# fonzcastellanos/scalable-video-codec

Measured on AMD Instinct MI355X. Metric: encoded frames/sec (1080p, 16x16 HBMA+DCT), higher is better.
Workload: dtype u8 (SAD, integer argmin) / f64 accumulate -> f32 (DCT, quant)

## Files before the change

include/svc/clip_encoder.hpp:

```cpp
#ifndef SVC_CLIP_ENCODER_HPP
#define SVC_CLIP_ENCODER_HPP

#include <cstdint>
#include <functional>
#include <memory>

#include "svc_hip.h"

namespace svc {

struct Shard {
  uint32_t first_frame = 0;
  uint32_t frames = 0;
  bool needs_halo = false;
  uint32_t pairs = 0;
  uint32_t first_encoded = 0;
};

Shard PlanShard(uint32_t clip_frames, uint32_t world, uint32_t rank);

enum class Schedule : uint32_t { kSerial = 0, kPipelined = 1 };

struct ClipEncoderConfig {
  uint32_t width = 0, height = 0;
  uint32_t levels = 3;
  uint32_t mv_block = 16;
  uint32_t search_range = 8;
  uint32_t dct_block_w = 8, dct_block_h = 8;
  uint32_t fg_step = 1, bg_step = 640;
  bool wire = false;
  bool compact = false;
  bool segmentation = true;
  uint64_t seed = 0;
  svc_ransac_params ransac{1, 7.5f, 0.99f, 0.5f};
  svc_segment_params segment{3, 3, 10, 3, 10, 1.0f, 4};
  uint32_t clip_frames = 0;
  uint32_t rank = 0, world = 1;
  Schedule schedule = Schedule::kPipelined;
  uint32_t hbma_flags = SVC_HBMA_AUTO;
  uint32_t lat_depth = 0;
  bool standalone_shapes = false;
  bool segment_fork = false;
  bool inline_rmse = false;
  bool narrow_attempts = false;
  bool two_bgr_passes = false;
  bool always_speculate = false;
  bool keep_foreground_prior = false;
  uint32_t chunk_pairs = 0;
  bool whole_shard_steps = false;
  bool idle_rule_any_size = false;
  bool fork_behind_front = false;
  bool random_policy = false;
  bool mixed_steps = false;
  bool search_after_transform = false;
};

enum class Stage : uint32_t { kLumaPyramid = 0, kHalo, kHbma, kRansac, kSegment, kTransform, kTypePatch, kCount };
enum class Buffer : uint32_t { kMv = 0, kMinMad, kGlobalMotion, kRmse, kInlierMask, kInlierCount, kBlockTypes,
                               kCoeffs, kRecords, kPyramids, kBgr,
                               kCompact , kCompactOffsets ,
                               kCompactChoice , kCount };

class ClipEncoder {
 public:
  using HaloFn = std::function<void(const uint8_t* d_send, uint8_t* d_recv, uint64_t bytes, void* stream)>;

  explicit ClipEncoder(const ClipEncoderConfig& config);
  ~ClipEncoder();
  ClipEncoder(const ClipEncoder&) = delete;
  ClipEncoder& operator=(const ClipEncoder&) = delete;

  const Shard& shard() const;
  uint32_t padded_width() const;
  uint32_t padded_height() const;
  uint32_t blocks() const;
  uint64_t pyramid_stride() const;

  void LoadFrames(const uint8_t* src, uint32_t first_local, uint32_t n, bool src_on_device);

  void SetComm(void* nccl_comm);
  void SetHaloTransport(HaloFn fn);

  void Step(bool timed = false);
  uint32_t StepFrames(const uint8_t* device_frames, bool timed = false);
  void WaitStep(uint32_t step);
  void SetCompactBudget(const svc_step_pair* ladder, uint32_t ladder_len, uint32_t bytes_per_frame);
  void Flush();
  void Sync();

  void StageTime(Stage s, double* total_ms, uint32_t* launches);
  uint64_t StagePairs(Stage s);
  void ResetTimers();
  uint32_t steps_submitted() const;
  uint32_t chunks_per_step() const;
  uint32_t output_sets() const;

  void ResetPolicy();
  void PolicyInfo(uint64_t* chunks_decided, uint64_t* chunks_speculated, double* foreground_share);

  void* Output(Buffer b, uint64_t* bytes);

 private:
  struct Impl;
  std::unique_ptr<Impl> p_;
  void StepOn(const uint8_t* frames, bool timed);
};

// ... 4 lines not shown
```

include/svc_clip.h:

```cpp
#ifndef SVC_CLIP_H
#define SVC_CLIP_H

#include <stdint.h>

#include "svc_hip.h"

#ifdef __cplusplus
extern "C" {
#endif

typedef struct svc_clip svc_clip;

#define SVC_CLIP_SERIAL 0u
#define SVC_CLIP_PIPELINED 1u

#define SVC_CLIP_TUNE_STANDALONE_SHAPES 1u
#define SVC_CLIP_TUNE_SEGMENT_FORK 2u
#define SVC_CLIP_TUNE_INLINE_RMSE 8u
#define SVC_CLIP_TUNE_NARROW_ATTEMPTS 4u
#define SVC_CLIP_TUNE_TWO_BGR_PASSES 16u
#define SVC_CLIP_TUNE_ALWAYS_SPECULATE 32u
#define SVC_CLIP_KEEP_FOREGROUND_PRIOR 64u
#define SVC_CLIP_OUTPUT_COMPACT 8192u
#define SVC_CLIP_TUNE_IDLE_RULE_ANY_SIZE 512u
#define SVC_CLIP_TUNE_FORK_BEHIND_FRONT 4096u
#define SVC_CLIP_TUNE_RANDOM_POLICY 2048u
#define SVC_CLIP_TUNE_MIXED_STEPS 1024u
#define SVC_CLIP_TUNE_SEARCH_AFTER_TRANSFORM 256u
#define SVC_CLIP_TUNE_WHOLE_SHARD_STEPS 128u

typedef struct svc_clip_config {
  uint32_t struct_size;
  uint32_t width, height;
  uint32_t levels, mv_block, search_range;
  uint32_t dct_block_w, dct_block_h;
  uint32_t fg_step, bg_step;
  uint32_t wire;
  uint32_t segmentation;
  uint64_t seed;
  svc_ransac_params ransac;
  svc_segment_params segment;
  uint32_t clip_frames;
  uint32_t rank, world;
  uint32_t schedule;
  uint32_t chunk_pairs;
  uint32_t hbma_flags;
  uint32_t lat_depth;
  uint32_t tuning;
} svc_clip_config;

typedef struct svc_clip_info {
  uint32_t padded_w, padded_h, mv_field_w, mv_field_h, blocks, ransac_iters;
  uint64_t pyramid_stride, frame_bytes, record_bytes;
  uint32_t first_frame, frames, pairs, first_encoded, needs_halo;
  uint32_t chunks_per_step;
  uint32_t output_sets;
  uint32_t reserved;
} svc_clip_info;

enum { SVC_STAGE_LUMA_PYRAMID = 0, SVC_STAGE_HALO, SVC_STAGE_HBMA, SVC_STAGE_RANSAC, SVC_STAGE_SEGMENT,
       SVC_STAGE_TRANSFORM, SVC_STAGE_TYPE_PATCH ,
       SVC_STAGE_COUNT };
enum { SVC_BUF_MV = 0, SVC_BUF_MIN_MAD, SVC_BUF_GLOBAL_MOTION, SVC_BUF_RMSE, SVC_BUF_INLIER_MASK,
       SVC_BUF_INLIER_COUNT, SVC_BUF_BLOCK_TYPES, SVC_BUF_COEFFS, SVC_BUF_RECORDS, SVC_BUF_PYRAMIDS,
       SVC_BUF_BGR, SVC_BUF_COMPACT , SVC_BUF_COMPACT_OFFSETS,
       SVC_BUF_COMPACT_CHOICE , SVC_BUF_COUNT };

typedef int (*svc_clip_halo_fn)(const uint8_t* d_send, uint8_t* d_recv, uint64_t bytes, void* stream,
                                void* user);

const char* svc_clip_last_error(void);

int svc_clip_plan_shard(uint32_t clip_frames, uint32_t world, uint32_t rank, uint32_t* first_frame,
                        uint32_t* frames, uint32_t* pairs, uint32_t* first_encoded);

int svc_clip_create(const svc_clip_config* config, svc_clip** out);
void svc_clip_destroy(svc_clip* clip);
int svc_clip_get_info(svc_clip* clip, svc_clip_info* out);

int svc_clip_load_frames(svc_clip* clip, const uint8_t* src, uint32_t first_local, uint32_t n,
                         int src_on_device);

// ... 27 lines not shown
```

scalable_video_codec_amd/clip.py:

```python
from __future__ import annotations

import ctypes as C
import os
from typing import Callable, Dict, Optional, Tuple

import torch

from . import native
from .configs import CodecConfig
from .native import RansacParams, SegmentParams

_vp, _u32, _u64 = C.c_void_p, C.c_uint32, C.c_uint64

SERIAL, PIPELINED = 0, 1
TUNE_STANDALONE_SHAPES, TUNE_SEGMENT_FORK, TUNE_NARROW_ATTEMPTS, TUNE_INLINE_RMSE, TUNE_TWO_BGR_PASSES, TUNE_ALWAYS_SPECULATE = 1, 2, 4, 8, 16, 32
TUNE_IDLE_RULE_ANY_SIZE = 512
TUNE_FORK_BEHIND_FRONT = 4096
TUNE_RANDOM_POLICY = 2048
TUNE_MIXED_STEPS = 1024
TUNE_SEARCH_AFTER_TRANSFORM = 256
TUNE_WHOLE_SHARD_STEPS = 128
OUTPUT_COMPACT = 8192
KEEP_FOREGROUND_PRIOR = 64
STAGES = ("luma_pyramid", "halo_exchange", "hbma", "ransac", "segment", "dct_quant", "type_patch")
BUFFERS = {"mv": (0, torch.float32), "min_mad": (1, torch.float32), "global_motion": (2, torch.float32),
           "rmse": (3, torch.float32), "inlier_mask": (4, torch.uint8), "inlier_count": (5, torch.int32),
           "block_types": (6, torch.int32), "coeffs": (7, torch.float32), "records": (8, torch.uint8),
           "pyramids": (9, torch.uint8), "bgr": (10, torch.uint8), "compact": (11, torch.uint8), "compact_offsets": (12, torch.int64),
           "compact_choice": (13, torch.int32)}
COMM_ID_BYTES = 128


class ClipConfig(C.Structure):
    _fields_ = [("struct_size", _u32), ("width", _u32), ("height", _u32), ("levels", _u32), ("mv_block", _u32), ("search_range", _u32),
                ("dct_block_w", _u32), ("dct_block_h", _u32), ("fg_step", _u32), ("bg_step", _u32), ("wire", _u32),
                ("segmentation", _u32), ("seed", _u64), ("ransac", RansacParams), ("segment", SegmentParams),
                ("clip_frames", _u32), ("rank", _u32), ("world", _u32), ("schedule", _u32), ("chunk_pairs", _u32),
                ("hbma_flags", _u32), ("lat_depth", _u32), ("tuning", _u32)]


class ClipInfo(C.Structure):
    _fields_ = [(n, _u32) for n in ("padded_w", "padded_h", "mv_field_w", "mv_field_h", "blocks", "ransac_iters")] + \
               [(n, _u64) for n in ("pyramid_stride", "frame_bytes", "record_bytes")] + \
               [(n, _u32) for n in ("first_frame", "frames", "pairs", "first_encoded", "needs_halo", "chunks_per_step", "output_sets", "reserved")]


HALO_FN = C.CFUNCTYPE(C.c_int, _vp, _vp, _u64, _vp, _vp)

SIGNATURES = {
    "svc_clip_last_error": (C.c_char_p, []),
    "svc_clip_plan_shard": (C.c_int, [_u32, _u32, _u32] + [C.POINTER(_u32)] * 4),
    "svc_clip_create": (C.c_int, [C.POINTER(ClipConfig), C.POINTER(_vp)]),
    "svc_clip_destroy": (None, [_vp]),
    "svc_clip_get_info": (C.c_int, [_vp, C.POINTER(ClipInfo)]),
    "svc_clip_load_frames": (C.c_int, [_vp, _vp, _u32, _u32, C.c_int]),
    "svc_clip_set_comm": (C.c_int, [_vp, _vp]),
    "svc_clip_set_halo_callback": (C.c_int, [_vp, HALO_FN, _vp]),
    "svc_clip_step": (C.c_int, [_vp, C.c_int]),
    "svc_clip_step_frames": (C.c_int, [_vp, _vp, C.c_int, C.POINTER(_u32)]),
    "svc_clip_wait_step": (C.c_int, [_vp, _u32]),
    "svc_clip_set_compact_budget": (C.c_int, [_vp, C.POINTER(native.StepPair), _u32, _u32]),
    "svc_clip_flush": (C.c_int, [_vp]),
    "svc_clip_sync": (C.c_int, [_vp]),
    "svc_clip_stage_time": (C.c_int, [_vp, _u32, C.POINTER(C.c_double), C.POINTER(_u32)]),
    "svc_clip_stage_pairs": (C.c_int, [_vp, _u32, C.POINTER(_u64)]),
    "svc_clip_reset_timers": (C.c_int, [_vp]),
    "svc_clip_reset_policy": (C.c_int, [_vp]),
    "svc_clip_policy_info": (C.c_int, [_vp, C.POINTER(_u64), C.POINTER(_u64), C.POINTER(C.c_double)]),
    "svc_clip_output": (C.c_int, [_vp, _u32, C.POINTER(_vp), C.POINTER(_u64)]),
    "svc_clip_read": (C.c_int, [_vp, _u32, _u64, _vp, _u64, C.c_int]),
}

_lib: Optional[C.CDLL] = None

# ... 211 lines not shown
```

scalable_video_codec_amd/csrc/host/clip_encoder.cpp:

```cpp
#include "svc/clip_encoder.hpp"

#include <algorithm>
#include <cstring>
#include <stdexcept>
#include <string>
#include <utility>
#include <vector>

#include "encode_geometry.hpp"
#include "hip_raii.hpp"
#include "svc_clip.h"

namespace svc {
namespace {

using namespace host;

constexpr Who kWho{"svc::ClipEncoder"};
void Hip(hipError_t e, const char* what) { kWho.Hip(e, what); }
void Abi(int rc, const char* what) { kWho.Abi(rc, what); }
bool Ready(hipEvent_t e) { return kWho.Ready(e); }

constexpr uint32_t kStages = (uint32_t)Stage::kCount;

}

Shard PlanShard(uint32_t clip_frames, uint32_t world, uint32_t rank) {
  Shard s;
  if (world == 0 || rank >= world) return s;
  const uint32_t base = clip_frames / world, extra = clip_frames % world;
  s.frames = base + (rank < extra ? 1u : 0u);
  s.first_frame = rank * base + std::min(rank, extra);
  s.needs_halo = s.first_frame > 0 && s.frames > 0;
  s.pairs = s.frames == 0 ? 0 : s.frames - (s.needs_halo ? 0u : 1u);
  s.first_encoded = s.needs_halo ? s.first_frame : s.first_frame + 1;
  return s;
}

struct ClipEncoder::Impl : EncodeGeometry {
  ClipEncoderConfig c;
  Shard sh;
  uint32_t iters = 0;
  uint64_t record_bytes = 0, seg_ws_bytes = 0;
  static constexpr int kMaxDepth = 3, kSets = kMaxDepth + 2;
  int depth = 1, nsets = 1;
  uint32_t nch = 1, cp = 0;
  struct Micro { uint32_t step = 0, p0 = 0, pn = 0; bool first = true; uint8_t order = 0; const uint8_t* frames = nullptr; };
  static constexpr int kRing = 8;
  Micro ring[kRing], next_micro;
  uint32_t n_steps = 0;
  const uint8_t* step_frames = nullptr;
  Event e_step[kRing];
  uint64_t step_last_micro[kRing] = {};
  void MarkStepDone(uint64_t d) {
    const uint32_t s = StepOf(d);
    if (step_last_micro[s % kRing] == d) Hip(hipEventRecord(e_step[s % kRing], sM), "hipEventRecord");
  }
  const Micro& At(uint64_t m) const { return ring[(int)(m % (uint64_t)kRing)]; }
  uint32_t StepOf(uint64_t m) const { return At(m).step; }
  uint32_t P0(uint64_t m) const { return At(m).p0; }
  uint32_t Pn(uint64_t m) const { return At(m).pn; }
  int Slot(uint64_t m) const { return (int)(m % (uint64_t)nsets); }
  DevBuf<uint8_t> bgr, pyr[2], mask[kSets], seg_ws[kMaxDepth], records[kSets + 1];
  DevBuf<float> mv[kSets], mad[kSets], gm[kSets], rmse[kSets], coeffs[kSets + 1];
  DevBuf<uint8_t> redo_ws[kMaxDepth];
  DevBuf<uint32_t> count[kSets], types[kSets], samples;
  DevBuf<uint8_t> compact, compact_ws;
  DevBuf<uint64_t> compact_off;
  std::vector<svc_step_pair> budget_ladder;
  DevBuf<uint32_t> compact_budget, compact_choice;
  Event e_pyr[2], e_halo[2], e_fork, e_join[kSets], e_rfork, e_rmse[kSets];
  bool halo_recorded[2] = {false, false}, join_pending[kSets] = {}, rmse_pending[kSets] = {};
  bool defer_rmse = false;
  uint64_t iter = 0, fork_iter[kSets] = {};
  void* comm = nullptr;
  HaloFn halo;
  uint64_t n_luma = 0, n_hbma = 0, n_lat = 0, n_dct = 0;
  uint32_t lat_flags = 0;
  bool fused_records = false;
  bool one_bgr_pass = false;
  int rec_sets = 1;
  DevBuf<uint8_t>& Records(uint64_t m) { return records[(int)(StepOf(m) % (uint32_t)rec_sets)]; }
  bool spec_quant = false;
  int coeff_sets = 1;
  DevBuf<float>& Coeffs(uint64_t m) { return coeffs[coeff_sets > 1 ? (int)(StepOf(m) % (uint32_t)coeff_sets) : 0]; }
  bool GrowCoeffSets() {
    if (coeff_sets == rec_sets) return true;
    while (n_dct < n_luma) Iterate(false, last_timed);
    for (int b = 1; b < rec_sets; ++b)
      if (!coeffs[b].TryAlloc(coeffs[0].n)) {
        for (int k = 1; k < b; ++k) coeffs[k].Free();
        spec_quant = false;
        return false;
      }
    coeff_sets = rec_sets;
    return true;
  }
  bool spec_step[kSets + 1] = {};
  bool& SpecStep(uint64_t m) { return spec_step[(int)(m % (uint64_t)(kSets + 1))]; }
  static constexpr int kFgSlots = 8;
  static constexpr double kSpecMaxShare = 0.02;
  static constexpr uint64_t kSpecMinPixels = 50000000ull;
  static constexpr uint64_t kChunkMinPixels = 300000000ull;
  static constexpr uint64_t kIdleRuleMinPixels = 400000000ull;
  static constexpr uint32_t kMaxAutoChunks = 1;
  DevBuf<uint32_t> fg_dev;
  PinBuf<uint32_t> fg_host;
  Event e_fg[kFgSlots];
  bool fg_pending[kFgSlots] = {};
  uint64_t fg_blocks[kFgSlots] = {};
  uint64_t n_fg = 0;
  double fg_share = -1.0;
  uint64_t n_spec = 0, n_decided = 0;
  void MeasureForeground(uint64_t m, hipStream_t st) {
    if (!spec_quant || c.two_bgr_passes || c.always_speculate || !Pn(m)) return;
    const int slot = (int)(n_fg % kFgSlots);
    if (fg_pending[slot] && !Ready(e_fg[slot])) return;
    Abi(svc_hip_count_foreground(types[Set(m)].p + (uint64_t)P0(m) * blocks, (uint64_t)Pn(m) * blocks, fg_dev.p + slot, st), "svc_hip_count_foreground");
    Hip(hipMemcpyAsync(fg_host.p + slot, fg_dev.p + slot, 4, hipMemcpyDeviceToHost, st), "hipMemcpyAsync");
    Hip(hipEventRecord(e_fg[slot], st), "hipEventRecord");
    fg_pending[slot] = true;
    fg_blocks[slot] = (uint64_t)Pn(m) * blocks;
    ++n_fg;
  }
  void PollForeground() {
// ... 22 lines not shown
  bool WouldReadOnce() {
    if (one_bgr_pass) return true;
    if (!spec_quant || c.two_bgr_passes) return false;
    if (c.always_speculate) return true;
    PollForeground();
    return fg_share >= 0.0 && fg_share <= kSpecMaxShare;
  }
  void ResetPolicy() {
    fg_share = -1.0;
    n_fg = 0;
    for (bool& p : fg_pending) p = false;
  }
  bool last_timed = false;
  std::vector<std::pair<Event, Event>> timed[kStages];
  std::vector<Event> event_pool;

  Event TimingEvent() {
    if (event_pool.empty()) return Event(kWho, true);
    Event e = std::move(event_pool.back());
    event_pool.pop_back();
    return e;
  }

  uint64_t timed_pairs[kStages] = {};
  uint64_t cur_pairs = 0;
  template <typename F> void Run(Stage st, hipStream_t stream, bool timing, F&& fn) {
    if (!timing) { fn(); return; }
    timed_pairs[(uint32_t)st] += cur_pairs;
    Event a = TimingEvent(), b = TimingEvent();
    Hip(hipEventRecord(a, stream), "hipEventRecord");
    fn();
    Hip(hipEventRecord(b, stream), "hipEventRecord");
    timed[(uint32_t)st].emplace_back(std::move(a), std::move(b));
  }

  int Par(uint64_t m) const { return c.schedule == Schedule::kPipelined ? (int)(StepOf(m) & 1u) : 0; }
  int Set(uint64_t m) const { return (int)(StepOf(m) % (uint32_t)nsets); }

  uint32_t Skip() const { return sh.needs_halo ? 0u : 1u; }
  bool decided = false;
  void Decide(uint64_t m) {
    if (At(m).order && spec_quant && Pn(m)) {
      decided = At(m).order == 2;
      ++n_decided;
      n_spec += decided;
      return;
    }
    decided = spec_quant && Pn(m) && DecideSpeculation(m);
    if (decided && coeff_sets != rec_sets && (!At(m).first || !GrowCoeffSets())) {
      decided = false;
      --n_spec;
    }
  }
  template <typename Between> void Luma(uint64_t m, hipStream_t st, bool timing, Between&& between) {
    cur_pairs = Pn(m);
    const int b = Par(m);
    const uint32_t p0 = P0(m), pn = Pn(m), skip = Skip();
    const bool first_chunk = At(m).first;
    if (spec_quant) SpecStep(m) = pn ? decided : false;
    if (pn && (one_bgr_pass || (spec_quant && SpecStep(m)))) {
      const uint8_t* enc = At(m).frames + (uint64_t)(skip + p0) * frame_bytes;
      uint8_t* slots = pyr[b].p + (uint64_t)(1 + skip + p0) * pyr_stride;
      Run(Stage::kTransform, st, timing, [&] {
        if (!one_bgr_pass)
          Abi(svc_hip_dct_quant_luma_frames(enc, frame_bytes, pn, pw, ph, c.dct_block_w, c.bg_step,
                                            Coeffs(m).p + (uint64_t)p0 * 3 * plane_elems, slots, pyr_stride, st), "svc_hip_dct_quant_luma_frames");
        else
          Abi(svc_hip_dct_records_luma_frames(enc, frame_bytes, pn, pw, ph, c.dct_block_w, ph,
                                              Records(m).p + (uint64_t)p0 * record_bytes, record_bytes, slots, pyr_stride, st), "svc_hip_dct_records_luma_frames");
      });
      between();
      cur_pairs = pn;
      Run(Stage::kLumaPyramid, st, timing, [&] {
        if (skip && first_chunk)
          Abi(svc_hip_luma_pyramid_frames(At(m).frames, frame_bytes, 1, pw, ph, c.levels, pyr[b].p + pyr_stride, pyr_stride, st),
              "svc_hip_luma_pyramid_frames");
        Abi(svc_hip_pyramid_levels_frames(slots, pyr_stride, pn, pw, ph, c.levels, st), "svc_hip_pyramid_levels_frames");
      });
      return;
    }
    const uint32_t f0 = first_chunk ? 0u : p0 + skip, f1 = p0 + pn + skip;
    if (f1 <= f0) return;
    Run(Stage::kLumaPyramid, st, timing, [&] {
      Abi(svc_hip_luma_pyramid_frames(At(m).frames + (uint64_t)f0 * frame_bytes, frame_bytes, f1 - f0, pw, ph, c.levels,
                                      pyr[b].p + (uint64_t)(1 + f0) * pyr_stride, pyr_stride, st), "svc_hip_luma_pyramid_frames");
    });
  }

  void Halo(uint64_t m, bool timing) {
    cur_pairs = 0;
    const int b = Par(m);
    Hip(hipEventRecord(e_pyr[b], sM), "hipEventRecord");
    Hip(hipStreamWaitEvent(sC, e_pyr[b], 0), "hipStreamWaitEvent");
    Run(Stage::kHalo, sC, timing, [&] {
      const uint8_t* send = pyr[b].p + (uint64_t)sh.frames * pyr_stride;
      if (halo) halo(send, pyr[b].p, pyr_stride, sC);
      else if (comm) Abi(svc_hip_halo_shift(comm, send, pyr[b].p, pyr_stride, c.rank, c.world, 0, sC), "svc_hip_halo_shift");
      else throw std::runtime_error("svc::ClipEncoder: world > 1 needs SetComm() or SetHaloTransport() before Step()");
    });
    Hip(hipEventRecord(e_halo[b], sC), "hipEventRecord");
    halo_recorded[b] = true;
  }

  void Hbma(uint64_t m, hipStream_t st, bool timing) {
    cur_pairs = Pn(m);
    const uint32_t p0 = P0(m), pn = Pn(m);
    if (!pn) return;
    const int b = Par(m), q = Set(m), k = Slot(m);
    const uint64_t t0 = (sh.needs_halo ? 0 : 1) + p0;
    if (rmse_pending[k]) {
      Hip(hipStreamWaitEvent(st, e_rmse[k], 0), "hipStreamWaitEvent");
      rmse_pending[k] = false;
    }
    Run(Stage::kHbma, st, timing, [&] {
      Abi(svc_hip_hbma_pairs(pyr[b].p + t0 * pyr_stride, pyr[b].p + (t0 + 1) * pyr_stride, pyr_stride, pn, c.levels, pw, ph,
                             c.search_range, c.mv_block, c.mv_block, mv[q].p + (uint64_t)p0 * blocks * 2, mad[q].p + (uint64_t)p0 * blocks,
                             c.hbma_flags, st), "svc_hip_hbma_pairs");
    });
  }

  void Lat(uint64_t m, hipStream_t st, bool timing) {
    cur_pairs = Pn(m);
    const uint32_t p0 = P0(m), pn = Pn(m);
    if (!pn) return;
    const int b = Set(m), k = Slot(m);
    DevBuf<uint8_t>& ws = seg_ws[c.schedule == Schedule::kPipelined ? (int)(m % (uint64_t)depth) : 0];
    const uint64_t g0 = sh.first_encoded - 1 + p0;
    float* gm_c = gm[b].p + (uint64_t)p0 * 2;
    float* rmse_c = rmse[b].p + p0;
    const float* mv_c = mv[b].p + (uint64_t)p0 * blocks * 2;
    uint8_t* mask_c = mask[b].p + (uint64_t)p0 * blocks;
    uint32_t* count_c = count[b].p + p0;
    uint32_t* types_c = types[b].p + (uint64_t)p0 * blocks;
    const uint32_t* samples_c = samples.p + (uint64_t)p0 * iters * c.ransac.subset_sz;
    Run(Stage::kRansac, st, timing, [&] {
      Hip(hipMemsetAsync(gm_c, 0, (size_t)pn * 2 * sizeof(float), st), "hipMemsetAsync");
      Abi(svc_hip_ransac_frames_ex(mv_c, blocks, pn, c.ransac, samples_c, iters, gm_c, rmse_c, mask_c, count_c,
                                   lat_flags | (defer_rmse ? SVC_LAUNCH_DEFER_RMSE : 0u), st), "svc_hip_ransac_frames");
    });
    if (defer_rmse && c.world == 1) {
      Hip(hipEventRecord(e_rfork, st), "hipEventRecord");
      Hip(hipStreamWaitEvent(sC, e_rfork, 0), "hipStreamWaitEvent");
      Abi(svc_hip_ransac_rmse_frames(mv_c, blocks, pn, c.ransac, gm_c, mask_c, count_c, rmse_c, sC), "svc_hip_ransac_rmse_frames");
      Hip(hipEventRecord(e_rmse[k], sC), "hipEventRecord");
      rmse_pending[k] = true;
    }
    Run(Stage::kSegment, st, timing, [&] {
      if (c.segmentation)
        Abi(svc_hip_segment_frames_ex(mask_c, mv_c, mfw, mfh, pn, c.mv_block, c.mv_block, c.segment,
                                      c.seed * 1000003ull + g0, ws.p, seg_ws_bytes, types_c, lat_flags, st),
            "svc_hip_segment_frames");
      else
        Abi(svc_hip_block_types_frames(mask_c, blocks, pn, types_c, st), "svc_hip_block_types_frames");
    });
    MeasureForeground(m, st);
    if (c.schedule == Schedule::kPipelined && OnePassStep(m)) FinishOnePass(m, st, timing);
  }

  bool OnePassStep(uint64_t m) { return Pn(m) && (one_bgr_pass || (spec_quant && SpecStep(m))); }

  void FinishOnePass(uint64_t m, hipStream_t st, bool timing) {
    cur_pairs = Pn(m);
    const uint32_t p0 = P0(m), pn = Pn(m);
    if (!pn || !c.dct_block_w) return;
    const int b = Set(m);
// ... 30 lines not shown
      else if (c.compact)
        Abi(svc_hip_dct_pack_levels_frames(enc, frame_bytes, pn, pw, ph, c.dct_block_w, types_c, c.mv_block, c.mv_block, c.fg_step, c.bg_step,
                                           compact_ws.p, compact_ws.bytes(), compact.p, compact.bytes(), compact_off.p, st),
            "svc_hip_dct_pack_levels_frames");
      else if (c.wire && fused_records)
        Abi(svc_hip_dct_records_frames(enc, frame_bytes, pn, pw, ph, c.dct_block_w, types_c, c.mv_block, c.mv_block,
                                       0, 0, ph, Records(m).p + (uint64_t)p0 * record_bytes, record_bytes, st), "svc_hip_dct_records_frames");
      else if (c.wire) {
        float* planes = coeffs[0].p + (uint64_t)p0 * 3 * plane_elems;
        Abi(svc_hip_dct_frames(enc, frame_bytes, pn, pw, ph, c.dct_block_w, c.dct_block_h, planes, st), "svc_hip_dct_frames");
        Abi(svc_hip_serialize_frames(planes, plane_elems, pn, types_c, pw, ph, c.dct_block_w, c.dct_block_h, mfw, mfh,
                                     c.mv_block, c.mv_block, Records(m).p + (uint64_t)p0 * record_bytes, record_bytes, st), "svc_hip_serialize_frames");
      } else
        Abi(svc_hip_dct_quant_frames(enc, frame_bytes, pn, pw, ph, c.dct_block_w, c.dct_block_h, types_c, c.mv_block,
                                     c.mv_block, c.fg_step, c.bg_step, Coeffs(m).p + (uint64_t)p0 * 3 * plane_elems, st), "svc_hip_dct_quant_frames");
    });
  }

  void ForkLat(uint64_t l, bool timing) {
    hipStream_t st = sL[l % (uint64_t)depth];
    Hip(hipEventRecord(e_fork, sM), "hipEventRecord");
    Hip(hipStreamWaitEvent(st, e_fork, 0), "hipStreamWaitEvent");
    Lat(l, st, timing);
    Hip(hipEventRecord(e_join[Slot(l)], st), "hipEventRecord");
    join_pending[Slot(l)] = true;
    fork_iter[Slot(l)] = iter;
    if (defer_rmse && c.world > 1 && Pn(l)) {
      const int b = Set(l);
      const uint32_t p0 = P0(l), pn = Pn(l);
      Abi(svc_hip_ransac_rmse_frames(mv[b].p + (uint64_t)p0 * blocks * 2, blocks, pn, c.ransac, gm[b].p + (uint64_t)p0 * 2,
                                     mask[b].p + (uint64_t)p0 * blocks, count[b].p + p0, rmse[b].p + p0, st), "svc_hip_ransac_rmse_frames");
      Hip(hipEventRecord(e_rmse[Slot(l)], st), "hipEventRecord");
      rmse_pending[Slot(l)] = true;
    }
  }
  void JoinLat(uint64_t l) {
    if (!join_pending[Slot(l)]) return;
    Hip(hipStreamWaitEvent(sM, e_join[Slot(l)], 0), "hipStreamWaitEvent");
    join_pending[Slot(l)] = false;
  }

  void Iterate(bool new_step, bool timing) {
    if (new_step) {
      ring[(int)(n_luma % (uint64_t)kRing)] = next_micro;
      Decide(n_luma);
    }
    const uint64_t lumas_before = n_luma, hbmas = n_hbma, lats = n_lat;
    const bool do_lat = n_lat < hbmas;
    const uint64_t l = n_lat, d = n_dct;
    const bool do_dct = n_dct < lats && (!new_step || iter - fork_iter[Slot(d)] >= (uint64_t)depth);
    const bool fork_late = c.fork_behind_front && c.world == 1 && new_step && next_micro.pn && (one_bgr_pass || (spec_quant && decided));
    if (do_lat && !fork_late) ForkLat(l, timing);
    const bool reorder = c.search_after_transform && c.world == 1;
    bool hbma_done = false;
    auto pending_searches = [&](uint64_t upto) {
      while (n_hbma < upto) { Hbma(n_hbma, sM, timing); ++n_hbma; }
    };
    if (new_step) {
      const uint64_t m = n_luma;
      const int b = Par(m);
      if (c.world > 1 && halo_recorded[b])
        Hip(hipStreamWaitEvent(sM, e_halo[b], 0), "hipStreamWaitEvent");
      Luma(m, sM, timing, [&] {
        if (do_lat && fork_late) ForkLat(l, timing);
        if (reorder) { pending_searches(lumas_before); hbma_done = true; }
      });
      if (c.world > 1) Halo(m, timing);
      ++n_luma;
    }
    if (reorder) {
      if (do_dct) { JoinLat(d); Transform(d, sM, timing); MarkStepDone(d); }
      if (!hbma_done) pending_searches(n_luma);
      n_lat += do_lat; n_dct += do_dct;
      ++iter;
      return;
    }
    const bool do_hbma = (c.world > 1 && new_step) ? n_hbma < lumas_before : n_hbma < n_luma;
    const uint64_t h = n_hbma;
    if (do_hbma && c.world > 1) Hip(hipStreamWaitEvent(sM, e_halo[Par(h)], 0), "hipStreamWaitEvent");
    if (do_hbma) Hbma(h, sM, timing);
    if (do_dct) {
      JoinLat(d);
      Transform(d, sM, timing);
      MarkStepDone(d);
    }
    n_hbma += do_hbma; n_lat += do_lat; n_dct += do_dct;
    ++iter;
  }

  void SerialStep(bool timing) {
    const uint64_t s = n_luma;
    ring[(int)(s % (uint64_t)kRing)] = Micro{n_steps++, 0u, sh.pairs, true, 0, step_frames};
    step_last_micro[(n_steps - 1) % kRing] = s;
    Decide(s);
    const int b = Par(s);
    if (c.world > 1 && halo_recorded[b]) Hip(hipStreamWaitEvent(sM, e_halo[b], 0), "hipStreamWaitEvent");
    Luma(s, sM, timing, [] {});
    if (c.world > 1) {
      Halo(s, timing);
      Hip(hipStreamWaitEvent(sM, e_halo[b], 0), "hipStreamWaitEvent");
    }
    Hbma(s, sM, timing);
    Lat(s, sM, timing);
    Transform(s, sM, timing);
    MarkStepDone(s);
    ++n_luma; ++n_hbma; ++n_lat; ++n_dct;
  }

  Stream sM, sL[kMaxDepth], sC;
};

ClipEncoder::ClipEncoder(const ClipEncoderConfig& config) : p_(new Impl) {
  Impl& m = *p_;
  m.c = config;
  const ClipEncoderConfig& c = m.c;
  if (!c.width || !c.height || !c.levels || c.levels > 16 || !c.mv_block || c.world == 0 || c.rank >= c.world)
    throw std::runtime_error("svc::ClipEncoder: invalid configuration");
  if (c.clip_frames < 2 || c.clip_frames < c.world)
    throw std::runtime_error("svc::ClipEncoder: a clip needs at least two frames and one frame per rank");
  if ((c.dct_block_w == 0) != (c.dct_block_h == 0))
    throw std::runtime_error("svc::ClipEncoder: transform block needs both sides");
  if (c.compact) {
    if (c.wire) throw std::runtime_error("svc::ClipEncoder: compact and wire are two different outputs: choose one");
    if (c.chunk_pairs) throw std::runtime_error("svc::ClipEncoder: compact needs whole-shard launches (chunk_pairs = 0): one launch per step makes the shard's frames one stream");
    if (c.dct_block_w != c.dct_block_h || (c.dct_block_w != 8 && c.dct_block_w != 16))
      throw std::runtime_error("svc::ClipEncoder: compact needs an 8x8 or 16x16 transform block");
    if (c.mv_block % c.dct_block_w != 0) throw std::runtime_error("svc::ClipEncoder: compact needs an MV block that is a multiple of the transform block");
    if (c.fg_step == 0 || c.bg_step == 0) throw std::runtime_error("svc::ClipEncoder: compact needs quant steps > 0");
  }
  m.sh = PlanShard(c.clip_frames, c.world, c.rank);
  if (c.schedule == Schedule::kPipelined) {
    if (!c.standalone_shapes) m.lat_flags |= SVC_LAUNCH_BESIDE;
    if (!c.segment_fork) m.lat_flags |= SVC_LAUNCH_NO_FORK;
  }
  if (c.narrow_attempts) m.lat_flags |= SVC_LAUNCH_NO_WIDE;
  if (c.lat_depth > (uint32_t)Impl::kMaxDepth) throw std::runtime_error("svc::ClipEncoder: lat_depth must be 0..3");
  static_cast<EncodeGeometry&>(m) = EncodeGeometry(c.width, c.height, c.levels, c.mv_block, c.mv_block);
  const bool transform = c.dct_block_w != 0;
  if (c.compact && m.pw % 16 != 0) throw std::runtime_error("svc::ClipEncoder: compact needs a padded width of whole 16-pixel segments");
  m.record_bytes = (c.wire && transform) ? svc_hip_serialized_frame_bytes(m.pw, m.ph, c.dct_block_w, c.dct_block_h) : 0;
  m.iters = svc_hip_ransac_iter_count(c.ransac);
  const uint32_t P = m.sh.pairs, N = m.sh.frames;
  const bool pipelined = c.schedule == Schedule::kPipelined;
  m.depth = 1;
  if (pipelined) m.depth = c.lat_depth ? (int)c.lat_depth : 2;
  m.nsets = !pipelined ? 1 : m.depth + 2;
  m.nch = 1;
  if (pipelined && c.world == 1 && P > 1) {
    if (c.chunk_pairs) m.nch = (P + c.chunk_pairs - 1) / c.chunk_pairs;
    else m.nch = (uint32_t)std::min<uint64_t>(Impl::kMaxAutoChunks, std::max<uint64_t>(1, (uint64_t)P * m.pw * m.ph / Impl::kChunkMinPixels));
    m.nch = std::min(m.nch, P);
  }
  m.cp = P ? (P + m.nch - 1) / m.nch : 0;
  if (m.cp) m.nch = (P + m.cp - 1) / m.cp;
  m.defer_rmse = pipelined && !c.inline_rmse && m.blocks > 8192;
  m.sM = Stream(kWho);
  m.sC = Stream(kWho);
  if (m.defer_rmse) {
    m.e_rfork = Event(kWho);
    for (int b = 0; b < m.nsets; ++b) m.e_rmse[b] = Event(kWho);
  }
  for (int k = 0; k < m.depth; ++k) m.sL[k] = Stream(kWho);
  for (Event* e : {&m.e_pyr[0], &m.e_pyr[1], &m.e_halo[0], &m.e_halo[1], &m.e_fork}) *e = Event(kWho);
  for (int b = 0; b < m.nsets; ++b) m.e_join[b] = Event(kWho);
  for (Event& e : m.e_step) e = Event(kWho);
  m.bgr.Alloc(kWho, (size_t)N * m.frame_bytes);
  for (int b = 0; b < (pipelined ? 2 : 1); ++b) {
    m.pyr[b].Alloc(kWho, (size_t)(N + 1) * m.pyr_stride);
    Hip(hipMemset(m.pyr[b].p, 0, (size_t)(N + 1) * m.pyr_stride), "hipMemset");
  }
  for (int b = 0; b < m.nsets; ++b) {
    m.mv[b].Alloc(kWho, (size_t)P * m.blocks * 2); m.mad[b].Alloc(kWho, (size_t)P * m.blocks);
    m.gm[b].Alloc(kWho, (size_t)P * 2); m.rmse[b].Alloc(kWho, P);
    m.mask[b].Alloc(kWho, (size_t)P * m.blocks); m.count[b].Alloc(kWho, P); m.types[b].Alloc(kWho, (size_t)P * m.blocks);
  }
  m.seg_ws_bytes = c.segmentation ? svc_hip_segment_workspace_bytes(m.mfw, m.mfh, std::max(m.cp, 1u), c.segment.attempt_count) : 0;
  for (int k = 0; k < m.depth; ++k) m.seg_ws[k].Alloc(kWho, m.seg_ws_bytes);
  m.fused_records = c.wire && c.dct_block_w == c.dct_block_h && c.dct_block_w <= 64 && c.dct_block_w % 2 == 0;
  m.one_bgr_pass = m.fused_records && !c.two_bgr_passes && transform && (c.dct_block_w == 8 || c.dct_block_w == 16) && m.pw % 16 == 0 &&
                   c.mv_block % c.dct_block_w == 0 && P > 0;
  m.spec_quant = !c.wire && !c.compact && !c.two_bgr_passes && transform && c.dct_block_w == c.dct_block_h && (c.dct_block_w == 8 || c.dct_block_w == 16) &&
                 m.pw % 16 == 0 && c.mv_block % 16 == 0 && c.mv_block % c.dct_block_w == 0 && c.fg_step > 0 && c.bg_step > 0 && P > 0 &&
                 (c.always_speculate || c.idle_rule_any_size || (uint64_t)P * m.pw * m.ph >= Impl::kSpecMinPixels);
  m.rec_sets = (m.one_bgr_pass || m.spec_quant) && pipelined ? (m.nsets + 1 + (int)m.nch - 1) / (int)m.nch : 1;
  if (transform) {
    if (c.wire)
      for (int b = 0; b < m.rec_sets; ++b) m.records[b].Alloc(kWho, (size_t)P * m.record_bytes);
    if (c.compact) {
      m.compact.Alloc(kWho, svc_hip_levels_max_bytes(P, m.pw, m.ph, c.dct_block_w, c.dct_block_h, c.mv_block, c.mv_block));
      m.compact_off.Alloc(kWho, (size_t)P + 1);
      m.compact_ws.Alloc(kWho, svc_hip_dct_pack_levels_workspace_bytes(P, m.pw, m.ph, c.dct_block_w, c.mv_block, c.mv_block));
    } else if (!c.wire || !m.fused_records)
      m.coeffs[0].Alloc(kWho, (size_t)P * 3 * m.plane_elems);
    if (m.spec_quant) {
      for (int k = 0; k < m.depth; ++k) m.redo_ws[k].Alloc(kWho, svc_hip_dct_redo_workspace_bytes(m.cp, m.pw, m.ph, c.mv_block, c.mv_block));
      m.fg_dev.Alloc(kWho, Impl::kFgSlots);
      m.fg_host.Alloc(kWho, Impl::kFgSlots);
      for (Event& e : m.e_fg) e = Event(kWho);
    }
  }
  {
    const size_t n = (size_t)P * m.iters * c.ransac.subset_sz;
    std::vector<uint32_t> h(std::max<size_t>(n, 1));
    FillRansacDraws(h.data(), m.sh.first_encoded - 1, P, m.iters, c.ransac.subset_sz, m.blocks, c.seed);
    m.samples.Alloc(kWho, n);
    if (n) Hip(hipMemcpy(m.samples.p, h.data(), n * sizeof(uint32_t), hipMemcpyHostToDevice), "hipMemcpy");
  }
  Hip(hipDeviceSynchronize(), "hipDeviceSynchronize");
}

ClipEncoder::~ClipEncoder() = default;
const Shard& ClipEncoder::shard() const { return p_->sh; }
uint32_t ClipEncoder::padded_width() const { return p_->pw; }
uint32_t ClipEncoder::padded_height() const { return p_->ph; }
uint32_t ClipEncoder::blocks() const { return p_->blocks; }
uint64_t ClipEncoder::pyramid_stride() const { return p_->pyr_stride; }
// ... 4 lines not shown
void ClipEncoder::ResetPolicy() {
  Sync();
  p_->ResetPolicy();
}

void ClipEncoder::PolicyInfo(uint64_t* chunks_decided, uint64_t* chunks_speculated, double* foreground_share) {
  Sync();
  p_->PollForeground();
  if (chunks_decided) *chunks_decided = p_->n_decided;
  if (chunks_speculated) *chunks_speculated = p_->n_spec;
  if (foreground_share) *foreground_share = p_->fg_share;
}

void ClipEncoder::LoadFrames(const uint8_t* src, uint32_t first_local, uint32_t n, bool src_on_device) {
  Impl& m = *p_;
  if (!src || (uint64_t)first_local + n > m.sh.frames) throw std::runtime_error("svc::ClipEncoder: LoadFrames out of range");
  Sync();
  if (!m.c.keep_foreground_prior) m.ResetPolicy();
  Hip(hipMemcpy(m.bgr.p + (size_t)first_local * m.frame_bytes, src, (size_t)n * m.frame_bytes,
                src_on_device ? hipMemcpyDeviceToDevice : hipMemcpyHostToDevice), "hipMemcpy");
  Hip(hipStreamSynchronize(nullptr), "hipStreamSynchronize");
}

void ClipEncoder::SetComm(void* nccl_comm) { p_->comm = nccl_comm; }
void ClipEncoder::SetHaloTransport(HaloFn fn) { p_->halo = std::move(fn); }

void ClipEncoder::Step(bool timed) { StepOn(p_->bgr.p, timed); }

uint32_t ClipEncoder::StepFrames(const uint8_t* device_frames, bool timed) {
  if (!device_frames) throw std::runtime_error("svc::ClipEncoder: StepFrames needs the shard's frames in device memory");
  if (reinterpret_cast<uintptr_t>(device_frames) % 16 != 0) throw std::runtime_error("svc::ClipEncoder: StepFrames: the frames must be 16-byte aligned");
  StepOn(device_frames, timed);
  return p_->n_steps - 1;
}

void ClipEncoder::WaitStep(uint32_t step) {
  Impl& m = *p_;
  if (step >= m.n_steps) throw std::runtime_error("svc::ClipEncoder: WaitStep of a step that has not been submitted");
  if (m.n_steps - step > (uint32_t)Impl::kRing) step = m.n_steps - (uint32_t)Impl::kRing;
  if (m.step_last_micro[step % Impl::kRing] >= m.n_dct) Flush();
  Hip(hipEventSynchronize(m.e_step[step % Impl::kRing]), "hipEventSynchronize");
}

void ClipEncoder::StepOn(const uint8_t* frames, bool timed) {
  Impl& m = *p_;
  m.last_timed = timed;
  m.step_frames = frames;
  if (m.c.schedule != Schedule::kPipelined) { m.SerialStep(timed); return; }
  const uint32_t P = m.sh.pairs;
  uint32_t n = m.nch, cp = m.cp;
  uint8_t order[2] = {0, 0};
  const bool idle = !m.c.chunk_pairs && !m.c.compact && m.c.world == 1 && !m.c.whole_shard_steps && m.n_dct == m.n_luma && P >= 2 &&
                    (m.c.idle_rule_any_size || (uint64_t)P * m.pw * m.ph >= Impl::kIdleRuleMinPixels);
  if (idle && !m.WouldReadOnce()) {
    n = 2; cp = (P + 1) / 2;
    if (m.spec_quant && !m.c.two_bgr_passes && m.c.mixed_steps && m.fg_share < 0.0) { order[0] = 1; order[1] = 2; }
  }
  for (uint32_t k = 0; k < n; ++k) {
    const uint32_t p0 = std::min(P, k * cp);
    m.next_micro = Impl::Micro{m.n_steps, p0, std::min(cp, P - p0), k == 0, n == 2 ? order[k] : (uint8_t)0, frames};
    if (k + 1 == n) m.step_last_micro[m.n_steps % Impl::kRing] = m.n_luma;
    m.Iterate(true, timed);
  }
  ++m.n_steps;
}

void ClipEncoder::SetCompactBudget(const svc_step_pair* ladder, uint32_t ladder_len, uint32_t bytes_per_frame) {
  Sync();
  Impl& m = *p_;
  const ClipEncoderConfig& c = m.c;
  if (!c.compact) throw std::runtime_error("svc::ClipEncoder: a byte budget is a setting of the compact stream (compact)");
  if (ladder_len == 0) { m.budget_ladder.clear(); return; }
  const uint32_t P = m.sh.pairs;
  Abi(svc_hip_dct_pack_levels_budget_frames(nullptr, m.frame_bytes, 0, m.pw, m.ph, c.dct_block_w, nullptr, c.mv_block, c.mv_block, ladder, ladder_len,
                                            nullptr, nullptr, ~0ull, nullptr, ~0ull, nullptr, nullptr, nullptr),
      "svc_hip_dct_pack_levels_budget_frames");
  if (!m.compact_budget.p) {
    m.compact_ws.Alloc(kWho, svc_hip_dct_pack_levels_budget_workspace_bytes(P, m.pw, m.ph, c.dct_block_w, c.mv_block, c.mv_block, 64));
    m.compact_budget.Alloc(kWho, std::max(P, 1u));
    m.compact_choice.Alloc(kWho, std::max(P, 1u));
    Hip(hipMemset(m.compact_choice.p, 0, m.compact_choice.bytes()), "hipMemset");
  }
  const std::vector<uint32_t> b(std::max(P, 1u), bytes_per_frame);
  Hip(hipMemcpy(m.compact_budget.p, b.data(), b.size() * sizeof(uint32_t), hipMemcpyHostToDevice), "hipMemcpy");
  m.budget_ladder.assign(ladder, ladder + ladder_len);
}

void ClipEncoder::Flush() {
  Impl& m = *p_;
  while (m.n_dct < m.n_luma) m.Iterate(false, m.last_timed);
}

void ClipEncoder::Sync() {
  Flush();
  for (const Stream* s : {&p_->sC, &p_->sL[0], &p_->sL[1], &p_->sL[2], &p_->sM})
    if (*s) Hip(hipStreamSynchronize(*s), "hipStreamSynchronize");
}

uint64_t ClipEncoder::StagePairs(Stage s) {
  Sync();
  return p_->timed_pairs[(uint32_t)s];
}

void ClipEncoder::StageTime(Stage s, double* total_ms, uint32_t* launches) {
  Sync();
  double t = 0;
  for (auto& pr : p_->timed[(uint32_t)s]) {
    float ms = 0;
    Hip(hipEventElapsedTime(&ms, pr.first, pr.second), "hipEventElapsedTime");
    t += ms;
  }
  if (total_ms) *total_ms = t;
  if (launches) *launches = (uint32_t)p_->timed[(uint32_t)s].size();
// ... 43 lines not shown
}

}

static_assert(sizeof(svc_clip_config) == 136 && sizeof(svc_clip_info) == 80, "the ctypes binding (clip.py) mirrors this layout");
struct svc_clip {
  std::unique_ptr<svc::ClipEncoder> enc;
  svc::ClipEncoderConfig cfg;
};

namespace {
thread_local std::string g_clip_err;

template <typename F> int Guard(F&& fn) {
  try {
    fn();
    return 0;
  } catch (const std::exception& e) {
    g_clip_err = e.what();
    return 1;
  } catch (...) {
    g_clip_err = "unknown exception";
    return 1;
  }
}
}

extern "C" {

const char* svc_clip_last_error(void) { return g_clip_err.c_str(); }

int svc_clip_plan_shard(uint32_t clip_frames, uint32_t world, uint32_t rank, uint32_t* first_frame, uint32_t* frames,
                        uint32_t* pairs, uint32_t* first_encoded) {
  return Guard([&] {
    if (world == 0 || rank >= world) throw std::runtime_error("svc_clip_plan_shard: rank out of range");
    const svc::Shard s = svc::PlanShard(clip_frames, world, rank);
    if (first_frame) *first_frame = s.first_frame;
    if (frames) *frames = s.frames;
    if (pairs) *pairs = s.pairs;
    if (first_encoded) *first_encoded = s.first_encoded;
  });
}

int svc_clip_create(const svc_clip_config* k, svc_clip** out) {
  return Guard([&] {
    if (!k || !out) throw std::runtime_error("svc_clip_create: null pointer");
    if (k->struct_size != sizeof(svc_clip_config))
      throw std::runtime_error("svc_clip_create: config->struct_size is " + std::to_string(k->struct_size) + ", this build's svc_clip_config has " +
                               std::to_string(sizeof(svc_clip_config)) + " bytes (set struct_size = sizeof(svc_clip_config))");
    constexpr uint32_t kHbmaBits = SVC_HBMA_FORCE_WAVE_PER_BLOCK | SVC_HBMA_FORCE_FUSED | SVC_HBMA_FORCE_TILED | SVC_HBMA_FORCE_LANE;
    constexpr uint32_t kTuneBits = SVC_CLIP_TUNE_STANDALONE_SHAPES | SVC_CLIP_TUNE_SEGMENT_FORK | SVC_CLIP_TUNE_NARROW_ATTEMPTS | SVC_CLIP_TUNE_INLINE_RMSE |
                                   SVC_CLIP_TUNE_TWO_BGR_PASSES | SVC_CLIP_TUNE_ALWAYS_SPECULATE | SVC_CLIP_KEEP_FOREGROUND_PRIOR |
                                   SVC_CLIP_TUNE_WHOLE_SHARD_STEPS | SVC_CLIP_TUNE_SEARCH_AFTER_TRANSFORM | SVC_CLIP_TUNE_IDLE_RULE_ANY_SIZE |
                                   SVC_CLIP_TUNE_MIXED_STEPS | SVC_CLIP_TUNE_RANDOM_POLICY | SVC_CLIP_TUNE_FORK_BEHIND_FRONT | SVC_CLIP_OUTPUT_COMPACT;
    if (k->hbma_flags & ~kHbmaBits) throw std::runtime_error("svc_clip_create: unknown hbma_flags bits");
    if (k->tuning & ~kTuneBits) throw std::runtime_error("svc_clip_create: unknown tuning bits");
    if (k->lat_depth > 3) throw std::runtime_error("svc_clip_create: lat_depth must be 0..3");
    if (k->schedule != SVC_CLIP_SERIAL && k->schedule != SVC_CLIP_PIPELINED) throw std::runtime_error("svc_clip_create: unknown schedule");
    svc::ClipEncoderConfig c;
    c.width = k->width; c.height = k->height; c.levels = k->levels; c.mv_block = k->mv_block;
    c.search_range = k->search_range; c.dct_block_w = k->dct_block_w; c.dct_block_h = k->dct_block_h;
    c.fg_step = k->fg_step; c.bg_step = k->bg_step; c.wire = k->wire != 0; c.segmentation = k->segmentation != 0;
    c.seed = k->seed; c.ransac = k->ransac; c.segment = k->segment; c.clip_frames = k->clip_frames;
    c.rank = k->rank; c.world = k->world;
    c.schedule = k->schedule == SVC_CLIP_SERIAL ? svc::Schedule::kSerial : svc::Schedule::kPipelined;
    c.hbma_flags = k->hbma_flags; c.lat_depth = k->lat_depth;
    c.standalone_shapes = (k->tuning & SVC_CLIP_TUNE_STANDALONE_SHAPES) != 0;
    c.segment_fork = (k->tuning & SVC_CLIP_TUNE_SEGMENT_FORK) != 0;
    c.narrow_attempts = (k->tuning & SVC_CLIP_TUNE_NARROW_ATTEMPTS) != 0;
    c.inline_rmse = (k->tuning & SVC_CLIP_TUNE_INLINE_RMSE) != 0;
    c.two_bgr_passes = (k->tuning & SVC_CLIP_TUNE_TWO_BGR_PASSES) != 0;
    c.always_speculate = (k->tuning & SVC_CLIP_TUNE_ALWAYS_SPECULATE) != 0;
    c.keep_foreground_prior = (k->tuning & SVC_CLIP_KEEP_FOREGROUND_PRIOR) != 0;
    c.whole_shard_steps = (k->tuning & SVC_CLIP_TUNE_WHOLE_SHARD_STEPS) != 0;
    c.search_after_transform = (k->tuning & SVC_CLIP_TUNE_SEARCH_AFTER_TRANSFORM) != 0;
    c.idle_rule_any_size = (k->tuning & SVC_CLIP_TUNE_IDLE_RULE_ANY_SIZE) != 0;
    c.mixed_steps = (k->tuning & SVC_CLIP_TUNE_MIXED_STEPS) != 0;
    c.random_policy = (k->tuning & SVC_CLIP_TUNE_RANDOM_POLICY) != 0;
    c.fork_behind_front = (k->tuning & SVC_CLIP_TUNE_FORK_BEHIND_FRONT) != 0;
    c.compact = (k->tuning & SVC_CLIP_OUTPUT_COMPACT) != 0;
    c.chunk_pairs = k->chunk_pairs;
    std::unique_ptr<svc_clip> h(new svc_clip);
    h->cfg = c;
    h->enc.reset(new svc::ClipEncoder(c));
    *out = h.release();
  });
}

void svc_clip_destroy(svc_clip* clip) { delete clip; }

int svc_clip_get_info(svc_clip* clip, svc_clip_info* o) {
  return Guard([&] {
    if (!clip || !o) throw std::runtime_error("svc_clip_get_info: null pointer");
    const svc::ClipEncoder& e = *clip->enc;
    const svc::Shard& s = e.shard();
    o->padded_w = e.padded_width(); o->padded_h = e.padded_height();
    o->mv_field_w = o->padded_w / clip->cfg.mv_block; o->mv_field_h = o->padded_h / clip->cfg.mv_block;
    o->blocks = e.blocks(); o->ransac_iters = svc_hip_ransac_iter_count(clip->cfg.ransac);
    o->pyramid_stride = e.pyramid_stride();
    o->frame_bytes = (uint64_t)o->padded_w * o->padded_h * 3;
    o->record_bytes = (clip->cfg.wire && clip->cfg.dct_block_w)
                          ? svc_hip_serialized_frame_bytes(o->padded_w, o->padded_h, clip->cfg.dct_block_w, clip->cfg.dct_block_h) : 0;
    o->first_frame = s.first_frame; o->frames = s.frames; o->pairs = s.pairs; o->first_encoded = s.first_encoded;
    o->needs_halo = s.needs_halo ? 1u : 0u;
    o->chunks_per_step = e.chunks_per_step();
    o->output_sets = e.output_sets();
    o->reserved = 0;
  });
}

int svc_clip_load_frames(svc_clip* clip, const uint8_t* src, uint32_t first_local, uint32_t n, int src_on_device) {
  return Guard([&] { clip->enc->LoadFrames(src, first_local, n, src_on_device != 0); });
}

int svc_clip_set_comm(svc_clip* clip, void* nccl_comm) { return Guard([&] { clip->enc->SetComm(nccl_comm); }); }

int svc_clip_set_halo_callback(svc_clip* clip, svc_clip_halo_fn fn, void* user) {
  return Guard([&] {
    if (!fn) { clip->enc->SetHaloTransport(nullptr); return; }
    clip->enc->SetHaloTransport([fn, user](const uint8_t* s, uint8_t* r, uint64_t bytes, void* stream) {
      if (fn(s, r, bytes, stream, user)) throw std::runtime_error("svc::ClipEncoder: the halo callback failed");
    });
  });
}

int svc_clip_step(svc_clip* clip, int timed) { return Guard([&] { clip->enc->Step(timed != 0); }); }
int svc_clip_step_frames(svc_clip* clip, const uint8_t* device_frames, int timed, uint32_t* step) {
  return Guard([&] {
    const uint32_t s = clip->enc->StepFrames(device_frames, timed != 0);
    if (step) *step = s;
  });
}
// ... 49 lines not shown
```

Baseline: 133,500.

## Run luma pyramid build on side stream concurrent with pending HBMA searches

For single-device pipelined runs with non-idle micro-steps, the pyramid-level kernels now go to a side stream (sC) after an event fork from the main stream. The main stream meanwhile issues the pending HBMA searches, and a later HBMA on that parity waits on the pyramid event. The aim is to overlap pyramid construction with motion search and remove serialization on the main stream. A tuning flag restores the old on-main behavior. The change adds event bookkeeping and risks the two stages contending for compute.

```diff
diff --git a/include/svc/clip_encoder.hpp b/include/svc/clip_encoder.hpp
--- a/include/svc/clip_encoder.hpp
+++ b/include/svc/clip_encoder.hpp
@@ -53,6 +53,7 @@
   bool random_policy = false;
   bool mixed_steps = false;
   bool search_after_transform = false;
+  bool pyramid_on_main = false;
 };
 
 enum class Stage : uint32_t { kLumaPyramid = 0, kHalo, kHbma, kRansac, kSegment, kTransform, kTypePatch, kCount };
diff --git a/include/svc_clip.h b/include/svc_clip.h
--- a/include/svc_clip.h
+++ b/include/svc_clip.h
@@ -28,6 +28,7 @@
 #define SVC_CLIP_TUNE_MIXED_STEPS 1024u
 #define SVC_CLIP_TUNE_SEARCH_AFTER_TRANSFORM 256u
 #define SVC_CLIP_TUNE_WHOLE_SHARD_STEPS 128u
+#define SVC_CLIP_TUNE_PYRAMID_ON_MAIN 16384u
 
 typedef struct svc_clip_config {
   uint32_t struct_size;
diff --git a/scalable_video_codec_amd/clip.py b/scalable_video_codec_amd/clip.py
--- a/scalable_video_codec_amd/clip.py
+++ b/scalable_video_codec_amd/clip.py
@@ -20,6 +20,7 @@
 TUNE_MIXED_STEPS = 1024
 TUNE_SEARCH_AFTER_TRANSFORM = 256
 TUNE_WHOLE_SHARD_STEPS = 128
+TUNE_PYRAMID_ON_MAIN = 16384
 OUTPUT_COMPACT = 8192
 KEEP_FOREGROUND_PRIOR = 64
 STAGES = ("luma_pyramid", "halo_exchange", "hbma", "ransac", "segment", "dct_quant", "type_patch")
diff --git a/scalable_video_codec_amd/csrc/host/clip_encoder.cpp b/scalable_video_codec_amd/csrc/host/clip_encoder.cpp
--- a/scalable_video_codec_amd/csrc/host/clip_encoder.cpp
+++ b/scalable_video_codec_amd/csrc/host/clip_encoder.cpp
@@ -45,7 +45,7 @@
   static constexpr int kMaxDepth = 3, kSets = kMaxDepth + 2;
   int depth = 1, nsets = 1;
   uint32_t nch = 1, cp = 0;
-  struct Micro { uint32_t step = 0, p0 = 0, pn = 0; bool first = true; uint8_t order = 0; const uint8_t* frames = nullptr; };
+  struct Micro { uint32_t step = 0, p0 = 0, pn = 0; bool first = true; uint8_t order = 0; const uint8_t* frames = nullptr; bool idle = false; };
   static constexpr int kRing = 8;
   Micro ring[kRing], next_micro;
   uint32_t n_steps = 0;
@@ -71,6 +71,10 @@
   DevBuf<uint32_t> compact_budget, compact_choice;
   Event e_pyr[2], e_halo[2], e_fork, e_join[kSets], e_rfork, e_rmse[kSets];
   bool halo_recorded[2] = {false, false}, join_pending[kSets] = {}, rmse_pending[kSets] = {};
+  bool co_run = false;
+  Event e_front;
+  uint64_t pyr_wait[2] = {0, 0};
+  bool CoRun(const Micro& mi, bool speculates) const { return co_run && mi.pn && !mi.idle && (one_bgr_pass || (spec_quant && speculates)); }
   bool defer_rmse = false;
   uint64_t iter = 0, fork_iter[kSets] = {};
   void* comm = nullptr;
@@ -199,7 +203,7 @@
       --n_spec;
     }
   }
-  template <typename Between> void Luma(uint64_t m, hipStream_t st, bool timing, Between&& between) {
+  template <typename Between> void Luma(uint64_t m, hipStream_t st, bool timing, bool side, Between&& between) {
     cur_pairs = Pn(m);
     const int b = Par(m);
     const uint32_t p0 = P0(m), pn = Pn(m), skip = Skip();
@@ -216,14 +220,26 @@
           Abi(svc_hip_dct_records_luma_frames(enc, frame_bytes, pn, pw, ph, c.dct_block_w, ph,
                                               Records(m).p + (uint64_t)p0 * record_bytes, record_bytes, slots, pyr_stride, st), "svc_hip_dct_records_luma_frames");
       });
-      between();
+      hipStream_t ps = st;
+      if (side) {
+        Hip(hipEventRecord(e_front, st), "hipEventRecord");
+        Hip(hipStreamWaitEvent(sC, e_front, 0), "hipStreamWaitEvent");
+        ps = sC;
+      } else {
+        between();
+      }
       cur_pairs = pn;
-      Run(Stage::kLumaPyramid, st, timing, [&] {
+      Run(Stage::kLumaPyramid, ps, timing, [&] {
         if (skip && first_chunk)
-          Abi(svc_hip_luma_pyramid_frames(At(m).frames, frame_bytes, 1, pw, ph, c.levels, pyr[b].p + pyr_stride, pyr_stride, st),
+          Abi(svc_hip_luma_pyramid_frames(At(m).frames, frame_bytes, 1, pw, ph, c.levels, pyr[b].p + pyr_stride, pyr_stride, ps),
               "svc_hip_luma_pyramid_frames");
-        Abi(svc_hip_pyramid_levels_frames(slots, pyr_stride, pn, pw, ph, c.levels, st), "svc_hip_pyramid_levels_frames");
+        Abi(svc_hip_pyramid_levels_frames(slots, pyr_stride, pn, pw, ph, c.levels, ps), "svc_hip_pyramid_levels_frames");
       });
+      if (side) {
+        Hip(hipEventRecord(e_pyr[m & 1], sC), "hipEventRecord");
+        pyr_wait[m & 1] = m + 1;
+        between();
+      }
       return;
     }
     const uint32_t f0 = first_chunk ? 0u : p0 + skip, f1 = p0 + pn + skip;
@@ -258,6 +274,10 @@
     if (rmse_pending[k]) {
       Hip(hipStreamWaitEvent(st, e_rmse[k], 0), "hipStreamWaitEvent");
       rmse_pending[k] = false;
+    }
+    if (pyr_wait[m & 1] == m + 1) {
+      Hip(hipStreamWaitEvent(st, e_pyr[m & 1], 0), "hipStreamWaitEvent");
+      pyr_wait[m & 1] = 0;
     }
     Run(Stage::kHbma, st, timing, [&] {
       Abi(svc_hip_hbma_pairs(pyr[b].p + t0 * pyr_stride, pyr[b].p + (t0 + 1) * pyr_stride, pyr_stride, pn, c.levels, pw, ph,
@@ -394,6 +414,7 @@
     const bool fork_late = c.fork_behind_front && c.world == 1 && new_step && next_micro.pn && (one_bgr_pass || (spec_quant && decided));
     if (do_lat && !fork_late) ForkLat(l, timing);
     const bool reorder = c.search_after_transform && c.world == 1;
+    const bool side = new_step && CoRun(next_micro, decided);
     bool hbma_done = false;
     auto pending_searches = [&](uint64_t upto) {
       while (n_hbma < upto) { Hbma(n_hbma, sM, timing); ++n_hbma; }
@@ -403,9 +424,9 @@
       const int b = Par(m);
       if (c.world > 1 && halo_recorded[b])
         Hip(hipStreamWaitEvent(sM, e_halo[b], 0), "hipStreamWaitEvent");
-      Luma(m, sM, timing, [&] {
+      Luma(m, sM, timing, side, [&] {
         if (do_lat && fork_late) ForkLat(l, timing);
-        if (reorder) { pending_searches(lumas_before); hbma_done = true; }
+        if (reorder || side) { pending_searches(lumas_before); hbma_done = true; }
       });
       if (c.world > 1) Halo(m, timing);
       ++n_luma;
@@ -417,16 +438,21 @@
       ++iter;
       return;
     }
-    const bool do_hbma = (c.world > 1 && new_step) ? n_hbma < lumas_before : n_hbma < n_luma;
-    const uint64_t h = n_hbma;
-    if (do_hbma && c.world > 1) Hip(hipStreamWaitEvent(sM, e_halo[Par(h)], 0), "hipStreamWaitEvent");
-    if (do_hbma) Hbma(h, sM, timing);
+    if (c.world == 1) {
+      if (!hbma_done) pending_searches(n_luma);
+    } else {
+      const bool do_hbma = new_step ? n_hbma < lumas_before : n_hbma < n_luma;
+      const uint64_t h = n_hbma;
+      if (do_hbma) Hip(hipStreamWaitEvent(sM, e_halo[Par(h)], 0), "hipStreamWaitEvent");
+      if (do_hbma) Hbma(h, sM, timing);
+      n_hbma += do_hbma;
+    }
     if (do_dct) {
       JoinLat(d);
       Transform(d, sM, timing);
       MarkStepDone(d);
     }
-    n_hbma += do_hbma; n_lat += do_lat; n_dct += do_dct;
+    n_lat += do_lat; n_dct += do_dct;
     ++iter;
   }
 
@@ -437,7 +463,7 @@
     Decide(s);
     const int b = Par(s);
     if (c.world > 1 && halo_recorded[b]) Hip(hipStreamWaitEvent(sM, e_halo[b], 0), "hipStreamWaitEvent");
-    Luma(s, sM, timing, [] {});
+    Luma(s, sM, timing, false, [] {});
     if (c.world > 1) {
       Halo(s, timing);
       Hip(hipStreamWaitEvent(sM, e_halo[b], 0), "hipStreamWaitEvent");
@@ -503,7 +529,8 @@
     for (int b = 0; b < m.nsets; ++b) m.e_rmse[b] = Event(kWho);
   }
   for (int k = 0; k < m.depth; ++k) m.sL[k] = Stream(kWho);
-  for (Event* e : {&m.e_pyr[0], &m.e_pyr[1], &m.e_halo[0], &m.e_halo[1], &m.e_fork}) *e = Event(kWho);
+  for (Event* e : {&m.e_pyr[0], &m.e_pyr[1], &m.e_halo[0], &m.e_halo[1], &m.e_fork, &m.e_front}) *e = Event(kWho);
+  m.co_run = pipelined && c.world == 1 && !c.pyramid_on_main && !m.defer_rmse;
   for (int b = 0; b < m.nsets; ++b) m.e_join[b] = Event(kWho);
   for (Event& e : m.e_step) e = Event(kWho);
   m.bgr.Alloc(kWho, (size_t)N * m.frame_bytes);
@@ -614,13 +641,14 @@
   uint8_t order[2] = {0, 0};
   const bool idle = !m.c.chunk_pairs && !m.c.compact && m.c.world == 1 && !m.c.whole_shard_steps && m.n_dct == m.n_luma && P >= 2 &&
                     (m.c.idle_rule_any_size || (uint64_t)P * m.pw * m.ph >= Impl::kIdleRuleMinPixels);
+  bool cut = false;
   if (idle && !m.WouldReadOnce()) {
-    n = 2; cp = (P + 1) / 2;
+    n = 2; cp = (P + 1) / 2; cut = true;
     if (m.spec_quant && !m.c.two_bgr_passes && m.c.mixed_steps && m.fg_share < 0.0) { order[0] = 1; order[1] = 2; }
   }
   for (uint32_t k = 0; k < n; ++k) {
     const uint32_t p0 = std::min(P, k * cp);
-    m.next_micro = Impl::Micro{m.n_steps, p0, std::min(cp, P - p0), k == 0, n == 2 ? order[k] : (uint8_t)0, frames};
+    m.next_micro = Impl::Micro{m.n_steps, p0, std::min(cp, P - p0), k == 0, n == 2 ? order[k] : (uint8_t)0, frames, cut};
     if (k + 1 == n) m.step_last_micro[m.n_steps % Impl::kRing] = m.n_luma;
     m.Iterate(true, timed);
   }
@@ -770,7 +798,8 @@
     constexpr uint32_t kTuneBits = SVC_CLIP_TUNE_STANDALONE_SHAPES | SVC_CLIP_TUNE_SEGMENT_FORK | SVC_CLIP_TUNE_NARROW_ATTEMPTS | SVC_CLIP_TUNE_INLINE_RMSE |
                                    SVC_CLIP_TUNE_TWO_BGR_PASSES | SVC_CLIP_TUNE_ALWAYS_SPECULATE | SVC_CLIP_KEEP_FOREGROUND_PRIOR |
                                    SVC_CLIP_TUNE_WHOLE_SHARD_STEPS | SVC_CLIP_TUNE_SEARCH_AFTER_TRANSFORM | SVC_CLIP_TUNE_IDLE_RULE_ANY_SIZE |
-                                   SVC_CLIP_TUNE_MIXED_STEPS | SVC_CLIP_TUNE_RANDOM_POLICY | SVC_CLIP_TUNE_FORK_BEHIND_FRONT | SVC_CLIP_OUTPUT_COMPACT;
+                                   SVC_CLIP_TUNE_MIXED_STEPS | SVC_CLIP_TUNE_RANDOM_POLICY | SVC_CLIP_TUNE_FORK_BEHIND_FRONT | SVC_CLIP_OUTPUT_COMPACT |
+                                   SVC_CLIP_TUNE_PYRAMID_ON_MAIN;
     if (k->hbma_flags & ~kHbmaBits) throw std::runtime_error("svc_clip_create: unknown hbma_flags bits");
     if (k->tuning & ~kTuneBits) throw std::runtime_error("svc_clip_create: unknown tuning bits");
     if (k->lat_depth > 3) throw std::runtime_error("svc_clip_create: lat_depth must be 0..3");
@@ -796,6 +825,7 @@
     c.mixed_steps = (k->tuning & SVC_CLIP_TUNE_MIXED_STEPS) != 0;
     c.random_policy = (k->tuning & SVC_CLIP_TUNE_RANDOM_POLICY) != 0;
     c.fork_behind_front = (k->tuning & SVC_CLIP_TUNE_FORK_BEHIND_FRONT) != 0;
+    c.pyramid_on_main = (k->tuning & SVC_CLIP_TUNE_PYRAMID_ON_MAIN) != 0;
     c.compact = (k->tuning & SVC_CLIP_OUTPUT_COMPACT) != 0;
     c.chunk_pairs = k->chunk_pairs;
     std::unique_ptr<svc_clip> h(new svc_clip);
```

Measured after the change: 135,800 (median of 6 runs). 1.7% higher.
